# AI-Unicamp/GestureDiffusion

Measured on AMD Instinct MI355X. Metric: denoised motion frames/sec (1000-step p_sample_loop, B=64, T=196, d=512), higher is better.
Workload: dtype f32; 1 GPU; BASELINE config 2: MDM_Old (V1 encoder-only topology) J=263 d=512 ff=1024 L=8 H=4, 1000-step p_sample_loop, batch 64/GPU x 196 frames, random weights, in-kernel Philox noise; global_batch=64, frames=196, parallelism=dp1 (independent samples, end-of-loop gather), step=one denoising step (forward + fused sampler update) over the rank's batch

## Files before the change

gesturediffusion_amd/csrc/gemm2.hip:

```cpp
#include "gdx_internal.h"
#include "gdx_device.h"

#include <cstdio>
#include <cstdlib>

namespace gdx {

__device__ __forceinline__ float erf_as(float x) {
    const float ax = fabsf(x);
    const float t = __frcp_rn(fmaf(0.3275911f, ax, 1.0f));
    float pl = fmaf(1.061405429f, t, -1.453152027f);
    pl = fmaf(pl, t, 1.421413741f);
    pl = fmaf(pl, t, -0.284496736f);
    pl = fmaf(pl, t, 0.254829592f);
    const float r = 1.0f - pl * t * __expf(-ax * ax);
    return copysignf(r, x);
}
__device__ __forceinline__ float gelu_fast(float x) { return x * 0.5f * (1.0f + erf_as(x * 0.70710678118654752440f)); }

__device__ __forceinline__ f32x2 gelu_fast2(f32x2 x) {
    const f32x2 z = x * 0.70710678118654752440f;
    const f32x2 ax = f32x2{fabsf(z.x), fabsf(z.y)};
    const f32x2 den = __builtin_elementwise_fma(f32x2{0.3275911f, 0.3275911f}, ax, f32x2{1.0f, 1.0f});
    const f32x2 t = f32x2{__frcp_rn(den.x), __frcp_rn(den.y)};
    f32x2 pl = __builtin_elementwise_fma(f32x2{1.061405429f, 1.061405429f}, t, f32x2{-1.453152027f, -1.453152027f});
    pl = __builtin_elementwise_fma(pl, t, f32x2{1.421413741f, 1.421413741f});
    pl = __builtin_elementwise_fma(pl, t, f32x2{-0.284496736f, -0.284496736f});
    pl = __builtin_elementwise_fma(pl, t, f32x2{0.254829592f, 0.254829592f});
    const f32x2 q = -ax * ax;
    const f32x2 ex = f32x2{__expf(q.x), __expf(q.y)};
    const f32x2 r = 1.0f - pl * t * ex;
    const f32x2 er = f32x2{copysignf(r.x, z.x), copysignf(r.y, z.y)};
    return x * 0.5f * (1.0f + er);
}

template <int R, int NRD, int NMM>
__device__ __forceinline__ void g4_sched_interleave() {
    if constexpr (R < NRD) {
        __builtin_amdgcn_sched_group_barrier(0x008, 1, 0);
        __builtin_amdgcn_sched_group_barrier(0x100, 1, 0);
        g4_sched_interleave<R + 1, NRD, NMM>();
    } else if constexpr (NMM > NRD) {
        __builtin_amdgcn_sched_group_barrier(0x008, NMM - NRD, 0);
    }
}

template <int MB, int NBW, int BK, int NST, bool RESP>
__global__ __launch_bounds__(512, 1) void gemm4_kernel(const GemmParams p, const int epi, const int omode, const int ntn,
                                                       const int ntiles, unsigned long long* dbg) {
#if defined(__HIP_DEVICE_COMPILE__)
    constexpr int BM = MB * 16, WN = NBW * 16, BN = WN * 4;
    constexpr int ST = BK + 8;
    constexpr int ROWB = ST * 4;
    constexpr int A_BYTES = (BM * ROWB + 1023) / 1024 * 1024;
    constexpr int W_BYTES = (BN * ROWB + 1023) / 1024 * 1024;
    constexpr int STAGE_BYTES = A_BYTES + W_BYTES;
    constexpr int A_P = A_BYTES / 1024, P = STAGE_BYTES / 1024;
    constexpr int PW = (P + 3) / 4;
    constexpr int KK = BK / 16;
    constexpr int NSTORE = MB * NBW * 4;
    constexpr int VM_STEP = NST >= 3 ? (NST - 3) * PW : 0;
    static_assert(W_BYTES == BN * ROWB, "W region must have no gap (rows past N are not padded)");
    static_assert(NST >= 2, "ring needs >= 2 stages");
    extern __shared__ __attribute__((aligned(16))) char smem[];
    float* const bias_lds = reinterpret_cast<float*>(smem + NST * STAGE_BYTES);

    const int tid = threadIdx.x;
    const int wave = __builtin_amdgcn_readfirstlane(tid) >> 6;
    const int lane = tid & 63;
    const int l15 = lane & 15, lq = lane >> 4;
    const int G = gridDim.x;
    const int lid = xcd_lid((int)blockIdx.x, G);
    const int my_tiles = lid < ntiles ? (ntiles - lid + G - 1) / G : 0;
    const int nk = p.K / BK;
    const int total = my_tiles * nk;
    if (total == 0) return;

    if (wave < 4)
        for (int i = tid; i < p.N; i += 256) bias_lds[i] = p.bias ? p.bias[i] : 0.0f;

    const auto rsrcA = __builtin_amdgcn_make_buffer_rsrc(const_cast<float*>(p.A), (short)0, 0x7ffffff0, 0x00020000);
    const auto rsrcW = __builtin_amdgcn_make_buffer_rsrc(const_cast<float*>(p.W), (short)0, 0x7ffffff0, 0x00020000);
    int voff[PW];
#pragma unroll
    for (int i = 0; i < PW; ++i) {
        int piece = (wave & 3) + 4 * i;
        piece = piece < P ? piece : P - 1;
        const bool isA = piece < A_P;
        const int o = (isA ? piece : piece - A_P) * 1024 + 16 * lane;
        const int row = o / ROWB;
        int c = (o % ROWB) / 16;
        c = c < BK / 4 ? c : 0;
        voff[i] = (row * (isA ? p.lda : p.ldw) + c * 4) * 4;
    }
    int ld_tile_i = 0, ld_ks = 0;
    int ld_m0 = (lid / ntn) * BM, ld_n0 = (lid % ntn) * BN;
    auto issue = [&](int stage) {
        const int a_so = (ld_m0 * p.lda + ld_ks * BK) * 4;
        const int w_so = (ld_n0 * p.ldw + ld_ks * BK) * 4;
        char* sb = smem + stage * STAGE_BYTES;
#pragma unroll
        for (int i = 0; i < PW; ++i) {
            int piece = (wave & 3) + 4 * i;
            piece = piece < P ? piece : P - 1;
            if (piece < A_P)
                __builtin_amdgcn_raw_ptr_buffer_load_lds(rsrcA, (lds_ptr_t)(sb + piece * 1024), 16, voff[i], a_so, 0, 0);
            else
                __builtin_amdgcn_raw_ptr_buffer_load_lds(rsrcW, (lds_ptr_t)(sb + A_BYTES + (piece - A_P) * 1024), 16,
                                                         voff[i], w_so, 0, 0);
        }
        asm volatile("" ::: "memory");
        if (++ld_ks == nk) {
            ld_ks = 0;
            ++ld_tile_i;
            const int ti = ld_tile_i < my_tiles ? ld_tile_i : my_tiles - 1;
            const int tile = lid + ti * G;
            ld_m0 = (tile / ntn) * BM;
            ld_n0 = (tile % ntn) * BN;
        }
    };

    if (wave >= 4) {
#pragma unroll
        for (int s = 0; s < NST - 1; ++s) issue(s);
        wait_vm<VM_STEP>();
        asm volatile("s_waitcnt lgkmcnt(0)\n\ts_barrier" ::: "memory");
        int wst = NST - 1;
        for (int g = 0; g < total; ++g) {
            issue(wst);
            wst = wst == NST - 1 ? 0 : wst + 1;
            wait_vm<VM_STEP>();
            asm volatile("s_barrier" ::: "memory");
        }
        wait_vm<0>();
        return;
    }

    f32x4 acc[MB][NBW];
#pragma unroll
    for (int i = 0; i < MB; ++i)
#pragma unroll
        for (int j = 0; j < NBW; ++j) acc[i][j] = f32x4{0.f, 0.f, 0.f, 0.f};
    const int a_off = l15 * ST + 4 * lq;
    const int b_off = A_BYTES / 4 + (wave * WN + l15) * ST + 4 * lq;
    f32x4 fa0[MB], fb0[NBW], fa1[MB], fb1[NBW];
    auto rd = [&](f32x4 (&fa)[MB], f32x4 (&fb)[NBW], int stage, int kk) {
        const float* S = reinterpret_cast<const float*>(smem + stage * STAGE_BYTES);
#pragma unroll
        for (int i = 0; i < MB; ++i) fa[i] = *reinterpret_cast<const f32x4*>(&S[a_off + i * 16 * ST + kk * 16]);
#pragma unroll
        for (int j = 0; j < NBW; ++j) fb[j] = *reinterpret_cast<const f32x4*>(&S[b_off + j * 16 * ST + kk * 16]);
    };
    auto mm = [&](const f32x4 (&fa)[MB], const f32x4 (&fb)[NBW]) {
#pragma unroll
        for (int e = 0; e < 4; ++e)
#pragma unroll
            for (int i = 0; i < MB; ++i)
#pragma unroll
                for (int j = 0; j < NBW; ++j)
                    acc[i][j] = __builtin_amdgcn_mfma_f32_16x16x4f32(fb[j][e], fa[i][e], acc[i][j], 0, 0, 0);
    };

    asm volatile("s_waitcnt lgkmcnt(0)\n\ts_barrier" ::: "memory");
    unsigned long long t0 = 0, r0 = 0;
    if (dbg) { t0 = __builtin_amdgcn_s_memtime(); r0 = __builtin_amdgcn_s_memrealtime(); }

    int ks = 0, stage = 0, tile_i = 0;
    rd(fa0, fb0, 0, 0);
    auto interleave = [&]() { g4_sched_interleave<0, MB + NBW, 4 * MB * NBW>(); };
    f32x4 radd[RESP ? MB : 1][RESP ? NBW : 1];
    auto load_res = [&](int tile) {
        if constexpr (RESP) {
            const int m0 = (tile / ntn) * BM, nl = (tile % ntn) * BN + wave * WN + 4 * lq;
#pragma unroll
            for (int i = 0; i < MB; ++i) {
                int m = m0 + i * 16 + l15;
                m = m < p.M ? m : p.M - 1;
                const float* rp = p.R + (long)m * p.ldr + nl;
#pragma unroll
                for (int j = 0; j < NBW; ++j) radd[i][j] = *reinterpret_cast<const f32x4*>(rp + j * 16);
            }
        }
    };
    load_res(lid);
    for (int g = 0; g < total; ++g) {
        const int nstage = stage == NST - 1 ? 0 : stage + 1;
        rd(fa1, fb1, stage, 1);
        mm(fa0, fb0);
        interleave();
        if (KK == 4) {
            rd(fa0, fb0, stage, 2);
            mm(fa1, fb1);
            interleave();
            rd(fa1, fb1, stage, 3);
            mm(fa0, fb0);
            interleave();
        }
        if constexpr (NST >= 3) rd(fa0, fb0, nstage, 0);
        mm(fa1, fb1);
        if constexpr (NST >= 3) interleave();
        if (++ks == nk) {
            ks = 0;
            const int tile = lid + tile_i * G;
            ++tile_i;
            const int m0 = (tile / ntn) * BM, n0 = (tile % ntn) * BN;
            const bool rowmap = omode == OUT_TOKROWS;
            const int nl = n0 + wave * WN + 4 * lq;
            if constexpr (RESP) {
                float* cp = p.C + (long)(m0 + l15) * p.ldc + nl;
#pragma unroll
                for (int j = 0; j < NBW; ++j) {
                    const f32x4 bv = *reinterpret_cast<const f32x4*>(&bias_lds[nl + j * 16]);
#pragma unroll
                    for (int i = 0; i < MB; ++i) {
                        *reinterpret_cast<f32x4*>(cp + (long)(i * 16) * p.ldc + j * 16) = (acc[i][j] + bv) + radd[i][j];
                        acc[i][j] = f32x4{0.f, 0.f, 0.f, 0.f};
                    }
                }
                if (g + 1 < total) load_res(lid + tile_i * G);
            } else if (!rowmap && !p.R && !p.V) {
                float* cp = p.C + (long)(m0 + l15) * p.ldc + nl;
#pragma unroll
                for (int j = 0; j < NBW; ++j) {
                    const f32x4 bv = *reinterpret_cast<const f32x4*>(&bias_lds[nl + j * 16]);
#pragma unroll
                    for (int i = 0; i < MB; ++i) {
                        f32x4 v = acc[i][j] + bv;
                        if (epi == EPI_GELU) {
                            const f32x2 lo = gelu_fast2(f32x2{v[0], v[1]}), hi = gelu_fast2(f32x2{v[2], v[3]});
                            v = f32x4{lo.x, lo.y, hi.x, hi.y};
                        }
                        *reinterpret_cast<f32x4*>(cp + (long)(i * 16) * p.ldc + j * 16) = v;
                        acc[i][j] = f32x4{0.f, 0.f, 0.f, 0.f};
                    }
                }
            } else {
                const bool need_b = rowmap || p.V != nullptr;
                f32x4 add[MB][NBW];
                long rows[MB];
#pragma unroll
                for (int i = 0; i < MB; ++i) {
                    int bs = 0;
                    if (need_b) {
                        const int mb0 = m0 + i * 16;
                        const int bb0 = mb0 / p.T, r = mb0 - bb0 * p.T + l15;
                        bs = p.T >= 16 ? bb0 + (r >= p.T ? 1 : 0) : bb0 + r / p.T;
                    }
                    const int m = m0 + i * 16 + l15;
                    rows[i] = m >= p.M ? -1L : rowmap ? (long)m + bs + 1 : (long)m;
#pragma unroll
                    for (int j = 0; j < NBW; ++j) {
                        f32x4 a = f32x4{0.f, 0.f, 0.f, 0.f};
                        if (rows[i] >= 0) {
                            if (p.R) a = *reinterpret_cast<const f32x4*>(&p.R[rows[i] * p.ldr + nl + j * 16]);
                            if (p.V) a += *reinterpret_cast<const f32x4*>(&p.V[(long)bs * p.ldv + nl + j * 16]);
                        }
                        add[i][j] = a;
                    }
                }
#pragma unroll
                for (int j = 0; j < NBW; ++j) {
                    const f32x4 bv = *reinterpret_cast<const f32x4*>(&bias_lds[nl + j * 16]);
#pragma unroll
                    for (int i = 0; i < MB; ++i) {
                        f32x4 v = (acc[i][j] + bv) + add[i][j];
                        if (epi == EPI_GELU) {
                            const f32x2 lo = gelu_fast2(f32x2{v[0], v[1]}), hi = gelu_fast2(f32x2{v[2], v[3]});
                            v = f32x4{lo.x, lo.y, hi.x, hi.y};
                        }
                        if (rows[i] >= 0) *reinterpret_cast<f32x4*>(&p.C[rows[i] * p.ldc + nl + j * 16]) = v;
                        acc[i][j] = f32x4{0.f, 0.f, 0.f, 0.f};
                    }
                }
            }
        }
        asm volatile("s_waitcnt lgkmcnt(0)\n\ts_barrier" ::: "memory");
        stage = nstage;
        if constexpr (NST == 2) rd(fa0, fb0, stage, 0);
    }
    if (dbg && blockIdx.x == 0 && tid == 0) {
        dbg[0] = __builtin_amdgcn_s_memtime() - t0;
        dbg[1] = __builtin_amdgcn_s_memrealtime() - r0;
        dbg[2] = (unsigned long long)total;
    }
#endif
}

template <int MB, int NBW, int BK, int NST>
constexpr size_t g4_lds_bytes(int N) {
    constexpr int ROWB = (BK + 8) * 4;
    constexpr int A_BYTES = (MB * 16 * ROWB + 1023) / 1024 * 1024, W_BYTES = (NBW * 64 * ROWB + 1023) / 1024 * 1024;
    return (size_t)NST * (A_BYTES + W_BYTES) + (size_t)N * 4;
}

template <int MB, int NBW, int BK, int NST, bool RESP = false>
static hipError_t launch_cfg(const GemmParams& p, int epi, int omode, int num_cus, hipStream_t s, GemmCtl* ctl) {
    if constexpr (!RESP && MB * NBW <= 10) {
        if (p.R && !p.V && omode == OUT_ROWS && epi == EPI_BIAS) return launch_cfg<MB, NBW, BK, NST, true>(p, epi, omode, num_cus, s, ctl);
    }
    constexpr int BM = MB * 16, BN = NBW * 64;
    static_assert(BM <= ROW_PAD, "whole-tile stores of the last row tile must stay inside the workspace padding");
    static_assert(g4_lds_bytes<MB, NBW, BK, NST>(1024) <= 160 * 1024, "tile does not fit the 160 KiB LDS");
    const size_t lds = g4_lds_bytes<MB, NBW, BK, NST>(p.N);
    static size_t attr_lds = 0;
    if (lds > attr_lds) {
        hipError_t e = hipFuncSetAttribute(reinterpret_cast<const void*>(&gemm4_kernel<MB, NBW, BK, NST, RESP>),
                                           hipFuncAttributeMaxDynamicSharedMemorySize, (int)lds);
        if (e != hipSuccess) return e;
        attr_lds = lds;
    }
    const int ntm = (p.M + BM - 1) / BM, ntn = p.N / BN;
    const int ntiles = ntm * ntn;
    const int grid = ntiles < num_cus ? ntiles : num_cus;
    if (ctl) ctl->ran = GemmLaunched{1, MB, NBW, BK, NST, RESP ? 1 : 0};
    hipLaunchKernelGGL((gemm4_kernel<MB, NBW, BK, NST, RESP>), dim3(grid), dim3(512), lds, s, p, epi, omode, ntn, ntiles,
                       ctl ? ctl->stamps : nullptr);
    return hipGetLastError();
}

#define G4_CONFIGS(X) \
    X(4, 2, 32, 4) X(5, 2, 32, 4) X(6, 2, 32, 4) X(8, 2, 32, 3) X(9, 2, 32, 3) X(5, 3, 32, 3) X(4, 3, 32, 3) X(4, 1, 64, 3) X(5, 1, 64, 3) X(4, 1, 32, 4) X(5, 1, 32, 4) X(8, 1, 32, 4) X(9, 1, 32, 4) X(2, 1, 64, 3) X(1, 1, 64, 3) X(5, 2, 64, 2) X(5, 3, 64, 2) X(4, 2, 64, 2) X(6, 2, 64, 2) X(8, 2, 64, 2) X(4, 3, 64, 2)

static bool g4_valid(int mb, int nbw, int bk, int nst, const GemmParams& p) {
    const size_t rowb = (size_t)(bk + 8) * 4;
    const size_t stage = (mb * 16 * rowb + 1023) / 1024 * 1024 + (nbw * 64 * rowb + 1023) / 1024 * 1024;
    return p.N % (nbw * 64) == 0 && p.K % bk == 0 && nst * stage + (size_t)p.N * 4 <= 160 * 1024;
}

static double g4_cost(int mb, int nbw, int bk, int M, int N, int K, int num_cus) {
    const int BM = mb * 16, BN = nbw * 64;
    const double tiles = (double)((M + BM - 1) / BM) * (N / BN);
    const double rounds = (double)(long)((tiles + num_cus - 1) / num_cus);
    const double mfma = (double)mb * nbw * (bk / 4) * 32.0;
    const double bytes = (double)(BM + BN) * bk * 4.0;
    const double mem = bytes / 14.0;
    const double step = (mfma > mem ? mfma : mem) + 150.0 + (mb + nbw) * (bk / 16) * 8.0;
    return rounds * ((K / bk) * step + mb * nbw * 4 * 12.0 + 300.0);
}

int gemm2_num_cus() {
    static int n = 0;
    if (!n) {
        int dev = 0;
        hipDeviceProp_t prop;
        if (hipGetDevice(&dev) == hipSuccess && hipGetDeviceProperties(&prop, dev) == hipSuccess)
            n = prop.multiProcessorCount;
        if (n <= 0) n = 256;
    }
    return n;
}

bool gemm2_supported(int omode, int epi, const GemmParams& p) {
    return (omode == OUT_ROWS || omode == OUT_TOKROWS) && (epi == EPI_BIAS || epi == EPI_GELU) && p.K % 32 == 0 && p.N % 64 == 0 && p.N <= 8192 && p.lda % 4 == 0 &&
           p.ldw % 4 == 0 && (long)(p.M + ROW_PAD) * p.lda * 4 < (1L << 31) && (long)(p.N + 128) * p.ldw * 4 < (1L << 31) &&
           p.ldc % 4 == 0 && ((uintptr_t)p.C & 15) == 0 && (!p.R || (p.ldr % 4 == 0 && ((uintptr_t)p.R & 15) == 0)) &&
           (!p.V || (p.ldv % 4 == 0 && ((uintptr_t)p.V & 15) == 0));
}

hipError_t launch_gemm2(int omode, int epi, const GemmParams& p, hipStream_t s, GemmCtl* ctl) {
    const int num_cus = gemm2_num_cus();
    int best_mb = 0, best_nbw = 0, best_bk = 0;
    static int force_mb = -1, force_nbw = -1, force_bk = -1;
    if (force_mb < 0) {
        force_mb = force_nbw = force_bk = 0;
        if (const char* e = getenv("GDX_GEMM_TILE")) sscanf(e, "%d,%d,%d", &force_mb, &force_nbw, &force_bk);
    }
    static const bool debug = getenv("GDX_GEMM_DEBUG") != nullptr;
    const bool forced = ctl && ctl->mb;
    const int f_mb = forced ? ctl->mb : force_mb, f_nbw = forced ? ctl->nbw : force_nbw, f_bk = forced ? ctl->bk : force_bk;
    double best = 1e30;
#define X(mb, nbw, bk, nst)                                                                       \
    if (g4_valid(mb, nbw, bk, nst, p) && !(nst == 2 && p.R)) {                            \
        double c = g4_cost(mb, nbw, bk, p.M, p.N, p.K, num_cus);                                  \
        if (f_mb == mb && f_nbw == nbw && f_bk == bk) c = 0.0;                                    \
        if (c < best) { best = c; best_mb = mb; best_nbw = nbw; best_bk = bk; }                   \
    }
    G4_CONFIGS(X)
#undef X
    if (!best_mb) return hipErrorNotSupported;
    if (debug)
        fprintf(stderr, "[gemm2] M=%d N=%d K=%d epi=%d -> tile %dx%d BK=%d\n", p.M, p.N, p.K, epi, best_mb * 16,
                best_nbw * 64, best_bk);
#define X(mb, nbw, bk, nst) \
    if (best_mb == mb && best_nbw == nbw && best_bk == bk) return launch_cfg<mb, nbw, bk, nst>(p, epi, omode, num_cus, s, ctl);
    G4_CONFIGS(X)
#undef X
    return hipErrorInvalidValue;
}

}
```

Before: 3091 frames/s.

## Hand-interleave LDS fragment reads with MFMAs using precomputed LDS address pointers

Replaces the sched_group_barrier interleave helper with explicit per-MFMA placement of the next k-slice's LDS fragment reads, fenced by sched_barrier. LDS addresses become precomputed address-space-3 lane pointers that are rebased per stage, which cuts per-read address arithmetic. For the two-stage pipeline, the stage barrier and first-fragment prefetch move inside the last MFMA group so the barrier overlaps the remaining MFMAs. The intent is to hide LDS latency and barrier stalls in the GEMM main loop. In exchange, the rigid scheduling can raise register pressure or serialise work badly if the placement is off.

```diff
diff --git a/gesturediffusion_amd/csrc/gemm2.hip b/gesturediffusion_amd/csrc/gemm2.hip
--- a/gesturediffusion_amd/csrc/gemm2.hip
+++ b/gesturediffusion_amd/csrc/gemm2.hip
@@ -32,17 +32,6 @@
     const f32x2 r = 1.0f - pl * t * ex;
     const f32x2 er = f32x2{copysignf(r.x, z.x), copysignf(r.y, z.y)};
     return x * 0.5f * (1.0f + er);
-}
-
-template <int R, int NRD, int NMM>
-__device__ __forceinline__ void g4_sched_interleave() {
-    if constexpr (R < NRD) {
-        __builtin_amdgcn_sched_group_barrier(0x008, 1, 0);
-        __builtin_amdgcn_sched_group_barrier(0x100, 1, 0);
-        g4_sched_interleave<R + 1, NRD, NMM>();
-    } else if constexpr (NMM > NRD) {
-        __builtin_amdgcn_sched_group_barrier(0x008, NMM - NRD, 0);
-    }
 }
 
 template <int MB, int NBW, int BK, int NST, bool RESP>
@@ -141,24 +130,38 @@
     for (int i = 0; i < MB; ++i)
 #pragma unroll
         for (int j = 0; j < NBW; ++j) acc[i][j] = f32x4{0.f, 0.f, 0.f, 0.f};
-    const int a_off = l15 * ST + 4 * lq;
-    const int b_off = A_BYTES / 4 + (wave * WN + l15) * ST + 4 * lq;
+    typedef const __attribute__((address_space(3))) char* lds_cptr;
+    typedef const __attribute__((address_space(3))) f32x4* lds_f4ptr;
+    lds_cptr a_lane = (lds_cptr)(lds_ptr_t)smem + (l15 * ST + 4 * lq) * 4;
+    lds_cptr b_lane = (lds_cptr)(lds_ptr_t)smem + A_BYTES + ((wave * WN + l15) * ST + 4 * lq) * 4;
+    asm volatile("" : "+v"(a_lane), "+v"(b_lane));
+    lds_cptr a_ad = a_lane, b_ad = b_lane;
+    auto to_stage = [&](int stage) {
+        a_ad = a_lane + stage * STAGE_BYTES;
+        b_ad = b_lane + stage * STAGE_BYTES;
+    };
     f32x4 fa0[MB], fb0[NBW], fa1[MB], fb1[NBW];
-    auto rd = [&](f32x4 (&fa)[MB], f32x4 (&fb)[NBW], int stage, int kk) {
-        const float* S = reinterpret_cast<const float*>(smem + stage * STAGE_BYTES);
-#pragma unroll
-        for (int i = 0; i < MB; ++i) fa[i] = *reinterpret_cast<const f32x4*>(&S[a_off + i * 16 * ST + kk * 16]);
-#pragma unroll
-        for (int j = 0; j < NBW; ++j) fb[j] = *reinterpret_cast<const f32x4*>(&S[b_off + j * 16 * ST + kk * 16]);
-    };
-    auto mm = [&](const f32x4 (&fa)[MB], const f32x4 (&fb)[NBW]) {
-#pragma unroll
-        for (int e = 0; e < 4; ++e)
+    auto rd1 = [&](f32x4 (&fa)[MB], f32x4 (&fb)[NBW], int kk, int r) {
+        if (r < MB) fa[r] = *(lds_f4ptr)(a_ad + r * 16 * ROWB + kk * 64);
+        else fb[r - MB] = *(lds_f4ptr)(b_ad + (r - MB) * 16 * ROWB + kk * 64);
+    };
+    auto rd = [&](f32x4 (&fa)[MB], f32x4 (&fb)[NBW], int kk) {
+#pragma unroll
+        for (int r = 0; r < MB + NBW; ++r) rd1(fa, fb, kk, r);
+    };
+    auto group = [&](const f32x4 (&fa)[MB], const f32x4 (&fb)[NBW], f32x4 (&na)[MB], f32x4 (&nb)[NBW], int kk_next, int e0 = 0,
+                     int e1 = 4) {
+#pragma unroll
+        for (int e = e0; e < e1; ++e)
 #pragma unroll
             for (int i = 0; i < MB; ++i)
 #pragma unroll
-                for (int j = 0; j < NBW; ++j)
+                for (int j = 0; j < NBW; ++j) {
                     acc[i][j] = __builtin_amdgcn_mfma_f32_16x16x4f32(fb[j][e], fa[i][e], acc[i][j], 0, 0, 0);
+                    const int n = (e * MB + i) * NBW + j;
+                    if (kk_next >= 0 && n < MB + NBW) rd1(na, nb, kk_next, n);
+                    __builtin_amdgcn_sched_barrier(0);
+                }
     };
 
     asm volatile("s_waitcnt lgkmcnt(0)\n\ts_barrier" ::: "memory");
@@ -166,8 +169,7 @@
     if (dbg) { t0 = __builtin_amdgcn_s_memtime(); r0 = __builtin_amdgcn_s_memrealtime(); }
 
     int ks = 0, stage = 0, tile_i = 0;
-    rd(fa0, fb0, 0, 0);
-    auto interleave = [&]() { g4_sched_interleave<0, MB + NBW, 4 * MB * NBW>(); };
+    rd(fa0, fb0, 0);
     f32x4 radd[RESP ? MB : 1][RESP ? NBW : 1];
     auto load_res = [&](int tile) {
         if constexpr (RESP) {
@@ -185,20 +187,29 @@
     load_res(lid);
     for (int g = 0; g < total; ++g) {
         const int nstage = stage == NST - 1 ? 0 : stage + 1;
-        rd(fa1, fb1, stage, 1);
-        mm(fa0, fb0);
-        interleave();
+        lds_cptr a_nx = a_ad, b_nx = b_ad;
+        if constexpr (NST == 2) {
+            a_nx = a_lane + nstage * STAGE_BYTES;
+            b_nx = b_lane + nstage * STAGE_BYTES;
+            asm volatile("" : "+v"(a_nx), "+v"(b_nx));
+            __builtin_amdgcn_sched_barrier(0);
+        }
+        group(fa0, fb0, fa1, fb1, 1);
         if (KK == 4) {
-            rd(fa0, fb0, stage, 2);
-            mm(fa1, fb1);
-            interleave();
-            rd(fa1, fb1, stage, 3);
-            mm(fa0, fb0);
-            interleave();
-        }
-        if constexpr (NST >= 3) rd(fa0, fb0, nstage, 0);
-        mm(fa1, fb1);
-        if constexpr (NST >= 3) interleave();
+            group(fa1, fb1, fa0, fb0, 2);
+            group(fa0, fb0, fa1, fb1, 3);
+        }
+        if constexpr (NST >= 3) {
+            to_stage(nstage);
+            group(fa1, fb1, fa0, fb0, 0);
+        } else {
+            group(fa1, fb1, fa0, fb0, -1, 0, 3);
+            asm volatile("s_waitcnt lgkmcnt(0)\n\ts_barrier" ::: "memory");
+            a_ad = a_nx; b_ad = b_nx;
+            rd(fa0, fb0, 0);
+            __builtin_amdgcn_sched_barrier(0);
+            group(fa1, fb1, fa0, fb0, -1, 3, 4);
+        }
         if (++ks == nk) {
             ks = 0;
             const int tile = lid + tile_i * G;
@@ -274,9 +285,8 @@
                 }
             }
         }
-        asm volatile("s_waitcnt lgkmcnt(0)\n\ts_barrier" ::: "memory");
+        if constexpr (NST >= 3) asm volatile("s_waitcnt lgkmcnt(0)\n\ts_barrier" ::: "memory");
         stage = nstage;
-        if constexpr (NST == 2) rd(fa0, fb0, stage, 0);
     }
     if (dbg && blockIdx.x == 0 && tid == 0) {
         dbg[0] = __builtin_amdgcn_s_memtime() - t0;
```

Result: faster. 3128 frames/s (median of 6 runs) (+1.2%).
